# jiaowoguanren0615/Segmentation_Factory

Measured on AMD Instinct MI355X. Metric: images/sec/GPU fwd+bwd SegFormer-B0 512x512 bf16; mIoU parity vs CPU ref, higher is better.
Workload: dtype bf16; 1 GPU; SegFormer-B0 (MiT-B0 + 768-wide SegFormerHead as the reference builds it), 150 classes, 512x512, full train step (zero_grad+fwd+CE/Dice+bwd+AGC/AdamW); per_gpu_batch=256, global_batch=256, parallelism=dp1, fp8=False, inputs=resident in HBM in the captured step's input buffers (zero-copy feed), launch=hipGraph(zero_grad+fwd+loss+bwd+grad gather) + RCCL all-reduce + fused AGC/AdamW

## Files before the change

### include/segfac.h

```cpp
#ifndef SEGFAC_H
#define SEGFAC_H
#include <stdint.h>

#ifdef __cplusplus
extern "C" {
#endif

#define SEGF_F32 0
#define SEGF_BF16 1
#define SEGF_ERR_SHAPE (-1)
#define SEGF_ERR_DTYPE (-2)
#define SEGF_ERR_WORKSPACE (-3)

const char* segf_version(void);

int segf_cast(const void* src, int src_dt, void* dst, int dst_dt, int64_t n, void* stream);
int segf_cast2d(const void* src, int src_dt, int64_t ld_src, void* dst, int dst_dt, int64_t ld_dst, int64_t rows, int64_t cols,
                void* stream);
int segf_permute021(const void* in, int in_dt, void* out, int out_dt, int64_t A, int64_t Bd, int64_t Cd,
                    int64_t ld_out, void* stream);
typedef struct SegfPrepItem {
    const void* src; void* dst;
    int64_t rows, cols, ld_src, ld_dst, pb, pc;
    int32_t op, src_dt, dst_dt, reserved;
// ... 105 lines not shown
int segf_bn_cls_bwd_supported(int dt, int64_t M, int C, int K, int64_t rows_per_sample);
int64_t segf_bn_cls_bwd_ws(int64_t M, int C, int64_t rows_per_sample);
int segf_bn_cls_bwd(int dt, int64_t M, int C, int K, const void* dy, int64_t ldy, const void* w, int64_t ldw, const void* x,
                    const float* mean, const float* rstd, const float* gamma, const float* beta, int act,
                    const float* chan_scale, int64_t rows_per_sample, int eval_mode, void* dx, float* dgamma, float* dbeta,
                    float* ws, void* stream);
int segf_bn_cls_bwd_dw_supported(int dt, int64_t M, int C, int K, int64_t rows_per_sample, int C1);
int64_t segf_bn_cls_bwd_dw_ws(int64_t M, int C, int64_t rows_per_sample);
int segf_bn_cls_bwd_dw(int dt, int64_t M, int C, int K, const void* dy, int64_t ldy, const void* w, int64_t ldw, const void* x,
                       const float* mean, const float* rstd, const float* gamma, const float* beta, int act,
                       const float* chan_scale, int64_t rows_per_sample, int eval_mode, void* dx, float* dgamma,
                       float* dbeta, float* ws, const void* x1, int64_t ldx1, int C1, float* dG, void* stream);
int64_t segf_bn_cls_bwd_full_ws(int64_t M, int C, int K, int64_t rows_per_sample);
int segf_bn_cls_bwd_full(int dt, int64_t M, int C, int K, const void* dy, int64_t ldy, const void* w, int64_t ldw, const void* x,
                         const float* mean, const float* rstd, const float* gamma, const float* beta, int act,
                         const float* chan_scale, int64_t rows_per_sample, int eval_mode, void* dx, float* dgamma, float* dbeta,
                         float* ws, const void* x1, int64_t ldx1, int C1, float* dG, float* dwcls, void* stream);

int64_t segf_grn_ws(int B, int64_t rows_per_sample, int C, int bwd);
int segf_grn_fwd(int dt, int B, int64_t rows_per_sample, int C, const void* x, const float* gamma, const float* beta, void* y,
                 float* a_scratch, float* sumsq_out, float* ws, int pre_gelu, void* stream);
int segf_grn_bwd(int dt, int B, int64_t rows_per_sample, int C, const void* x, const void* dy, const float* gamma,
                 const float* sumsq_saved, void* dx, float* dgamma, float* dbeta, float* ws, int pre_gelu, void* stream);

int segf_attention_fwd(int dt, int B, int heads, int N, int Nkv, int hd, const void* q, int64_t ldq,
                       const void* k, int64_t ldk, const void* v, int64_t ldv, float scale,
                       void* o, int64_t ldo, float* lse, void* stream);
int64_t segf_attention_bwd_ws(int B, int heads, int N, int Nkv, int hd);
int segf_attention_bwd(int dt, int B, int heads, int N, int Nkv, int hd, const void* q, int64_t ldq,
                       const void* k, int64_t ldk, const void* v, int64_t ldv, float scale,
                       const void* o, int64_t ldo, const void* d_o, int64_t lddo, const float* lse,
                       void* dq, int64_t lddq, void* dk, int64_t lddk, void* dv, int64_t lddv,
                       float* ws, void* stream);

int segf_group_attention_supported(int dt, int B, int H, int W, int heads, int hd, int G, int interval, int lda);
int segf_group_attention_fwd(int dt, int B, int H, int W, int heads, int hd, int G, int interval, int lda, const void* qkv,
                             int64_t ldqkv, const float* bias, float scale, void* o, int64_t ldo, float* lse, void* stream);
int64_t segf_group_attention_bwd_ws(int B, int H, int W, int heads, int hd, int G, int interval, int lda);
int segf_group_attention_bwd(int dt, int B, int H, int W, int heads, int hd, int G, int interval, int lda, const void* qkv,
                             int64_t ldqkv, const float* bias, float scale, const void* d_o, int64_t lddo, const float* lse,
                             void* dqkv, int64_t lddqkv, float* dbias, float* ws, void* stream);

int segf_dwconv3x3_gelu_fwd(int dt, int B, int H, int W, int C, const void* x, const float* w ,
                            const float* bias, int apply_gelu, void* y, void* stream);
int64_t segf_dwconv3x3_bwd_ws(int B, int H, int W, int C);
int segf_dwconv3x3_bwd_blocks(int dt, int B, int H, int W, int C);
int segf_dwconv3x3_gelu_bwd(int dt, int B, int H, int W, int C, const void* x, const float* w, const float* bias,
                            int apply_gelu, const void* dy, void* du, void* dx, float* dw, float* db,
                            float* ws, void* stream);
int segf_dwconv3x3_gelu_bwd_fc2_supported(int dt, int B, int H, int W, int C_hidden, int C_in);
int segf_dwconv3x3_gelu_bwd_fc2(int dt, int B, int H, int W, int C_hidden, int C_in, const void* f, const float* w9,
                                const float* bias, const void* dys, int64_t ld_dys, const void* w2, void* du, void* dx,
                                float* dw, float* db, float* ws, void* stream);

int segf_dwconv7x7_fwd(int dt, int B, int H, int W, int C, const void* x, const float* wt, const float* bias, void* y,
                       void* stream);
int64_t segf_dwconv7x7_bwd_ws(int B, int H, int W, int C);
int segf_dwconv7x7_bwd(int dt, int B, int H, int W, int C, const void* x, const float* wt, const void* dy, void* dx,
                       float* dw, float* db, float* ws, void* stream);

int segf_conv3x3_fwd_splitk(int mode, int B, int H, int W, int Cin, int Cout);
int segf_conv3x3_pick_splitk(int Cin, int Cout, int64_t P);
int segf_conv3x3(int mode, int B, int H, int W, int Cin, int Cout, const void* x, int64_t ldx, const void* w, int64_t ldw,
                 void* y, int y_dt, int64_t ldy, const float* bias, int split_k, float* ws, void* stream);

int segf_conv3x3_dil_live_taps(int H, int W, int dilation, int* taps );
int segf_conv3x3_dil_supported(int dt, int mode, int B, int H, int W, int Cin, int Cout, int dilation);
int segf_conv3x3_dil_pick_splitk(int B, int H, int W, int Cin, int Cout, int dilation);
int segf_conv3x3_dil(int dt, int mode, int B, int H, int W, int Cin, int Cout, int dilation, const void* x, int64_t ldx,
                     const void* w, int64_t ldw, void* y, int64_t ldy, int split_k, float* ws, void* stream);

int segf_gelu(int dt, int mode, const void* u, const void* dy, void* y, int64_t n, void* stream);
int segf_rowdot(const float* a, int64_t lda, const float* b, int64_t ldb, const float* extra_a, const float* extra_b,
                float* out, int64_t rows, int64_t cols, void* stream);
int segf_adaptive_avgpool(int dt, int bwd, int B, int H, int W, int C, int S, const void* in, void* out, void* stream);

int segf_im2col(int dt, int in_nchw_f32, int B, int H, int W, int Cin, int kh, int kw, int stride, int pad,
                int Ho, int Wo, const void* x, void* col, int64_t ldcol, void* stream);
int segf_col2im(int dt, int B, int H, int W, int Cin, int kh, int kw, int stride, int pad,
                int Ho, int Wo, const void* dcol, int64_t ldcol, void* dx, void* stream);

int segf_bilinear_fwd(int dt, int B, int h, int w, int C, const void* in, int64_t ldi,
                      int H, int W, void* out, int64_t ldo, int align_corners, void* stream);
int segf_bilinear_bwd(int dt, int B, int h, int w, int C, void* din, int64_t ldi,
                      int H, int W, const void* dout, int64_t ldo, int align_corners, void* stream);
int segf_bilinear_bwd_248(int dt, int B, int H, int W, int C, const void* dout, int64_t ldo, void* d2, void* d4, void* d8,
                          void* stream);
int segf_upsample_add(int dt, int B, int H, int W, int C, const void* base, int64_t ldb, int nsrc,
                      const void* src0, int h0, int w0, int64_t ld0, const void* src1, int h1, int w1, int64_t ld1,
                      const void* src2, int h2, int w2, int64_t ld2, void* out, int64_t ldo, int align_corners, void* stream);
int64_t segf_upsample_add_stats_ws(int B, int H, int W, int C);
int segf_upsample_add_stats(int dt, int B, int H, int W, int C, const void* base, int64_t ldb, int nsrc,
                            const void* src0, int h0, int w0, int64_t ld0, const void* src1, int h1, int w1, int64_t ld1,
                            const void* src2, int h2, int w2, int64_t ld2, void* out, int64_t ldo, int align_corners,
                            float* sums, float* ws, void* stream);
int segf_fuse_map_248_supported(int dt, int B, int H, int W, int C, int C1);
int64_t segf_fuse_map_248_ws(int B, int H, int W, int C);
int segf_fuse_map_248(int B, int H, int W, int C, int C1, const void* x1, int64_t ldx1, const void* g1, int64_t ldg,
                      const void* t2, int64_t ld2, const void* t3, int64_t ld3, const void* t4, int64_t ld4,
                      void* out, int64_t ldo, float* sums, float* ws, void* stream);
int segf_bn_stats_from_sums(const float* sums, int64_t rows, int C, float* mean, float* rstd, float* running_mean,
                            float* running_var, float momentum, float eps, void* stream);
int segf_nearest_up(int dt, int bwd, int B, int h, int w, int C, int H, int W, const void* in, const void* base, void* out,
                    void* stream);
int segf_bilinear_to_nchw_f32(int dt, int B, int h, int w, int C, const void* in, int64_t ldi,
                              int H, int W, float* out, void* stream);
// ... 70 lines not shown
```

### segmentation_factory_amd/csrc/conv.hip

```cpp
#include <stdlib.h>
#include "colreduce.h"

#define DW_PIX 4

template <typename T, int MODE>
__global__ void __launch_bounds__(256) dwconv3x3_kernel(const T* __restrict__ x, const float* __restrict__ w,
                                                         const float* __restrict__ bias, int apply_gelu,
                                                         const T* __restrict__ dy, T* __restrict__ y, int B, int H, int W, int C) {
    const int nchunk = C / 8;
    const int wg = (W + DW_PIX - 1) / DW_PIX;
    const int units = B * H * wg;
    const int64_t g = (int64_t)xcd_block() * 256 + threadIdx.x;
    const int ustep = (int)(((int64_t)gridDim.x * 256) / nchunk);
    const int c0 = (int)(g % nchunk) * 8;
    f32x2_t wk[9][4], bs[4];
#pragma unroll
    for (int jj = 0; jj < 4; ++jj) {
#pragma unroll
        for (int kk = 0; kk < 9; ++kk) {
            const int ks = MODE == 1 ? 8 - kk : kk;
            wk[kk][jj] = f32x2_t{w[(c0 + 2 * jj) * 9 + ks], w[(c0 + 2 * jj + 1) * 9 + ks]};
        }
        bs[jj] = (MODE != 1 && bias) ? f32x2_t{bias[c0 + 2 * jj], bias[c0 + 2 * jj + 1]} : f32x2_t{0.f, 0.f};
    }
// ... 311 lines not shown
                load_row(yin + 2, rawb[(j + 2) % 3]);
                load_grow(yin + 1, dysb[(j + 2) % 3]);
                const bool vy = yin >= 0 && yin < H && yin <= yb;
#pragma unroll
                for (int cx = 0; cx < DW_PIX + 2; ++cx) {
                    f32x2_t v[2];
                    unpack4v(curc[cx], vy && cok[cx], v);
#pragma unroll
                    for (int kx = 0; kx < 3; ++kx) {
                        const int p = cx - kx;
                        if (p >= 0 && p < DW_PIX) {
#pragma unroll
                            for (int jj = 0; jj < 2; ++jj) {
                                P[p][jj] = wk[6 + kx][jj] * v[jj] + P[p][jj];
                                Cc[p][jj] = wk[3 + kx][jj] * v[jj] + Cc[p][jj];
                                N[p][jj] = wk[kx][jj] * v[jj] + N[p][jj];
                            }
                        }
                    }
                }
                const int yo = yin - 1;
                if (yo >= ya && yo < yb) {
                    dwf_f32x4 dgf[4];
#pragma unroll
                    for (int jm = 0; jm < 4; ++jm) {
                        dgf[jm] = dwf_f32x4{0.f, 0.f, 0.f, 0.f};
#pragma unroll
                        for (int s = 0; s < KS; ++s)
                            dgf[jm] = __builtin_amdgcn_mfma_f32_16x16x32_bf16(__builtin_bit_cast(dwf_bf16x8, gcurc[s]), Bf[jm][s], dgf[jm], 0, 0, 0);
                    }
                    T* orow = yo_b + (int64_t)yo * W * C;
#pragma unroll
                    for (int h = 0; h < DW_PIX / 2; ++h) {
                        f32x2_t a8[4] = {P[2 * h][0], P[2 * h][1], P[2 * h + 1][0], P[2 * h + 1][1]};
                        Raw4<T> q0, q1;
                        q0.u.x = pack2bf(dgf[0][2 * h], dgf[1][2 * h]); q0.u.y = pack2bf(dgf[2][2 * h], dgf[3][2 * h]);
                        q1.u.x = pack2bf(dgf[0][2 * h + 1], dgf[1][2 * h + 1]); q1.u.y = pack2bf(dgf[2][2 * h + 1], dgf[3][2 * h + 1]);
                        f32x2_t gy[4], g0[2], g1[2];
                        unpack4v(q0, true, g0); unpack4v(q1, true, g1);
                        gy[0] = g0[0]; gy[1] = g0[1]; gy[2] = g1[0]; gy[3] = g1[1];
                        gelu_erf8<true>(a8, gy);
                        const f32x2_t o0[2] = {a8[0], a8[1]}, o1[2] = {a8[2], a8[3]};
                        if (cok[2 * h + 1]) store4v(orow + coff[2 * h + 1], o0);
                        if (cok[2 * h + 2]) store4v(orow + coff[2 * h + 2], o1);
                    }
                }
#pragma unroll
                for (int p = 0; p < DW_PIX; ++p) { P[p][0] = bs[0]; P[p][1] = bs[1]; }
            }
        }
    }
}

static inline int dw_blocks(int B, int H, int W, int C) {
    return colfixed_blocks((int64_t)B * H * ((W + DW_PIX - 1) / DW_PIX), C / 8, 8, 16384);
}

extern "C" int segf_dwconv3x3_gelu_fwd(int dt, int B, int H, int W, int C, const void* x, const float* w, const float* bias,
                                       int apply_gelu, void* y, void* stream) {
    if (B <= 0 || H <= 0 || W <= 0) return 0;
    if (C <= 0 || C % 8 != 0 || ((uintptr_t)x % 16) || ((uintptr_t)y % 16)) return SEGF_ERR_SHAPE;
    if ((int64_t)B * H * W >= (1ll << 31)) return SEGF_ERR_SHAPE;
    hipStream_t st = (hipStream_t)stream;
    const int blocks = dw_blocks(B, H, W, C);
    SEGF_DISPATCH_DT(dt, T, {
        if (dw_use_walk()) dw_walk_launch<T, 0>(st, (const T*)x, w, bias, apply_gelu, (const T*)nullptr, (T*)y, B, H, W, C);
        else
        hipLaunchKernelGGL((dwconv3x3_kernel<T, 0>), dim3(blocks), dim3(256), 0, st, (const T*)x, w, bias, apply_gelu,
                           (const T*)nullptr, (T*)y, B, H, W, C);
    })
    SEGF_CHECK_LAUNCH();
    return 0;
}

#define DWG_MAX_BLOCKS 1024
struct DwgPlan { int ch, rl, slabs, nblk, units_per_blk; };
static inline DwgPlan dwg_plan(int B, int H, int W, int C) {
    DwgPlan p;
    const int nchunk = C / 8;
    p.ch = nchunk < 256 ? nchunk : 256;
    p.rl = 256 / p.ch;
    p.slabs = (nchunk + p.ch - 1) / p.ch;
    const int64_t units = (int64_t)B * H * ((W + DW_PIX - 1) / DW_PIX);
    int64_t want = cdiv64(units, (int64_t)p.rl * 4);
    int cap = DWG_MAX_BLOCKS / p.slabs;
    if (cap < 1) cap = 1;
    p.nblk = (int)(want < 1 ? 1 : (want > cap ? cap : want));
    p.units_per_blk = (int)cdiv64(units, p.nblk);
    return p;
}

template <typename T>
__global__ void __launch_bounds__(256) dwconv3x3_wgrad_kernel(const T* __restrict__ x, const T* __restrict__ du,
                                                               float* __restrict__ partial, int B, int H, int W, int C, int ch,
                                                               int rl, int units_per_blk) {
    __shared__ float red[256 * 8];
    const int tx = threadIdx.x % ch, ty = threadIdx.x / ch;
    const int chunk = blockIdx.y * ch + tx;
    const int c0 = chunk * 8;
    const bool active = ty < rl && c0 < C;
    const int wg = (W + DW_PIX - 1) / DW_PIX;
    const int units = B * H * wg;
    float acc[10][8];
#pragma unroll
    for (int o = 0; o < 10; ++o)
#pragma unroll
        for (int j = 0; j < 8; ++j) acc[o][j] = 0.f;
    (void)units_per_blk;
    if (active) {
        for (int u = (int)xcd_block() * rl + ty; u < units; u += (int)gridDim.x * rl) {
            const int xg = u % wg;
            const int t = u / wg;
            const int yy = t % H;
            const int b = t / H;
            const int x0 = xg * DW_PIX;
            Raw8<T> graw[DW_PIX], vraw[3][DW_PIX + 2];
#pragma unroll
            for (int p = 0; p < DW_PIX; ++p) {
                const int xp = x0 + p < W ? x0 + p : W - 1;
                graw[p] = load8_raw<T>(du + (((int64_t)b * H + yy) * W + xp) * C + c0);
            }
#pragma unroll
            for (int ky = 0; ky < 3; ++ky) {
// ... 955 lines not shown
```

### segmentation_factory_amd/csrc/policy.h

```cpp
#pragma once

#define SEGF_POLICY_TABLE(X)                                                                                                             \
                                                                                                   \
    X(gemm_no_big, "SEGFAC_GEMM_NO_BIG", 0, "never take the 256 x 256-tile kernel (gemm_bf16_big_kernel): everything on the 128-tile one") \
    X(gemm_no_skinny, "SEGFAC_GEMM_NO_SKINNY", 0, "no streaming products for K, N <= 128 (gemm_skinny_kernel and its relatives)")        \
    X(gemm_no_skinny_rows, "SEGFAC_GEMM_NO_SKINNY_ROWS", 0, "the [tokens x 32] -> 768 projection on gemm_skinny_kernel instead of the whole-row form") \
    X(gemm_no_skinny_k, "SEGFAC_GEMM_NO_SKINNY_K", 0, "no K-split streaming product for 32- / 64-wide outputs (gemm_skinny_k_kernel)")  \
    X(gemm_no_dw_skinny, "SEGFAC_GEMM_NO_DW_SKINNY", 0, "small-output weight gradients on the tiled split-K kernel instead of gemm_dw_skinny_kernel") \
    X(gemm_no_narrow, "SEGFAC_GEMM_NO_NARROW", 0, "256-tile kernel: full 128 x 64 wave tiles also for outputs <= 160 wide (bit-identical results)") \
    X(gemm_no_deep, "SEGFAC_GEMM_NO_DEEP", 0, "256-tile forward: one K step of operand loads in flight instead of two")                  \
    X(gemm_no_deep128, "SEGFAC_GEMM_NO_DEEP128", 0, "128-tile kernel: one K step in flight instead of two")                              \
    X(gemm_no_fastload, "SEGFAC_GEMM_NO_FASTLOAD", 0, "guarded tile loads everywhere (no workgroup-uniform guard-free full-K-step loads)") \
    X(gemm_no_tr, "SEGFAC_GEMM_NO_TR", 0, "debugging: reduction-major fragments by scalar LDS reads instead of ds_read_b64_tr_b16; disables every kernel built on the transposed read") \
    X(gemm_no_pro, "SEGFAC_GEMM_NO_PRO", 0, "segf_gemm_pro_supported answers 0: BatchNorm + ReLU + Dropout2d are applied by their own pass") \
    X(gemm_no_fused_db, "SEGFAC_GEMM_NO_FUSED_DB", 0, "bias gradient as its own column-sum launch instead of riding on the weight-gradient product") \
    X(no_grouped_dw, "SEGFAC_NO_GROUPED_DW", 0, "segf_gemm_dw_db_grouped runs its members one by one")                                   \
    X(dw_no_xcd_slabs, "SEGFAC_DW_NO_XCD_SLABS", 0, "split-K weight gradients (128-tile kernel) in hardware workgroup order instead of one K slab per XCD")                \
    X(dw_no_shared_split, "SEGFAC_DW_NO_SHARED_SPLIT", 0, "grouped weight gradients keep their per-layer slice counts (also read by the host layer)") \
    X(no_wide_reduce, "SEGFAC_NO_WIDE_REDUCE", 0, "split-K partials of large outputs summed by the 16 x 16 form instead of whole rows")   \
    X(no_reduce4, "SEGFAC_NO_REDUCE4", 0, "split-K reduce: one output per thread instead of four (bitwise the same sums)")               \
    X(gemm_f32_no_mfma, "SEGFAC_GEMM_F32_NO_MFMA", 0, "fp32 storage (exact-parity mode, evaluate): products on the vector FMA kernel instead of the f32 matrix instruction") \
    X(gemm8_linear, "SEGFAC_GEMM8_LINEAR", 1, "0: plain nn.Linear products never take the eight-phase kernel (the 256 / 128 tile kernels as in r04)") \
    X(gemm8_linear_min_tiles, "SEGFAC_GEMM8_LINEAR_MIN_TILES", 128, "fewest 256 x 256 tiles for which a K >= 2048 nn.Linear product takes the eight-phase kernel (192 for shorter K)") \
    X(gemm8_linear_min_fill, "SEGFAC_GEMM8_LINEAR_MIN_FILL", 60, "smallest share (percent) of the launched 256 x 256 tiles that must be output for an nn.Linear product with ragged last tiles to take the eight-phase kernel") \
    X(gemm8_linear_min_k, "SEGFAC_GEMM8_LINEAR_MIN_K", 256, "shortest reduction for which an nn.Linear product takes the eight-phase kernel (its 12-load prologue and drain against K / 64 tiles)") \
    X(gemm8_dw, "SEGFAC_GEMM8_DW", 1, "0: nn.Linear weight gradients never take the eight-phase kernel below 65536 tokens (the grouped 128-tile kernel as in r04)") \
    X(gemm8_dw_min_gflop, "SEGFAC_GEMM8_DW_MIN_GFLOP", 100, "smallest nn.Linear weight gradient (GFLOP; both feature counts multiples of 256, >= 256 FLOP per operand byte) that takes the eight-phase kernel + a column-sum pass instead of the grouped 128-tile kernel") \
    X(gemm8_linear_min_gflop, "SEGFAC_GEMM8_LINEAR_MIN_GFLOP", 36, "smallest nn.Linear product (GFLOP, K >= 512; 100 for shorter K) that takes the eight-phase kernel") \
                                 \
    X(no_gemm8, "SEGFAC_NO_GEMM8", 0, "no eight-phase kernel at all (gemm8_kernel): the two-phase 256-tile kernel everywhere")           \
    X(no_gemm8t, "SEGFAC_NO_GEMM8T", 0, "no eight-phase kernel for weight gradients (reduction-major operands)")                         \
    X(conv_no_fwd_split, "SEGFAC_CONV_NO_FWD_SPLIT", 0, "3 x 3 forward / data gradient with few output tiles: no split over the (channel block, tap) walk") \
    X(g8_stagger, "SEGFAC_G8_STAGGER", -1, "eight-phase kernel: 1 = wave groups one barrier apart, 0 = lockstep, -1 = staggered for bf16 and the per-device choice (segf_gemm8_option) for fp8") \
    X(no_fp8, "SEGFAC_NO_FP8", 0, "segf_gemm_fp8_supported answers 0 (block-scaled 128-tile fp8 GEMM)")                                  \
    X(no_fp8_conv, "SEGFAC_NO_FP8_CONV", 0, "segf_conv3x3_fp8*_supported answer 0")                                                      \
    X(no_fp8_wgrad, "SEGFAC_NO_FP8_WGRAD", 0, "fp8 3 x 3 convolutions keep a bf16 weight gradient")                                      \
    X(no_fp8_linear, "SEGFAC_NO_FP8_LINEAR", 0, "segf_linear_fp8_supported answers 0")                                                   \
                                                                             \
    X(dilconv_no_cull, "SEGFAC_DILCONV_NO_CULL", 0, "dilated 3 x 3 convolution: all nine taps are walked, with zero loads where a tap leaves the image, instead of the live taps only") \
                                                                            \
    X(attn_no_mfma, "SEGFAC_ATTN_NO_MFMA", 0, "attention on the VALU reference kernels (attention.hip) also in bf16")                    \
    X(attn_f32_no_mfma, "SEGFAC_ATTN_F32_NO_MFMA", 0, "fp32 attention forward on the vector kernel (one query per lane) instead of the f32 matrix instruction") \
    X(attn64_prescale, "SEGFAC_ATTN64_PRESCALE", 0, "head dim 64, >= 128 keys: scale log2(e) rides on the Q fragments (bf16(q c), one more rounding per q element) and -max / -lse are the score accumulators' initial values, instead of one multiply-add per score: forward + query-side backward, +8 % / +2 % per kernel, attention error x 1.2 - 2.3") \
    X(attn64_dkv_rows, "SEGFAC_ATTN64_DKV_ROWS", 128, "head dim 64, >= 128 keys, key-side backward: query rows per staged Q / dO tile and barrier (128, 64 or 32: the same arithmetic, bit for bit)") \
    X(attn_no_fused_bwd, "SEGFAC_ATTN_NO_FUSED_BWD", 0, "head dim 32, <= 256 keys: query-side + key-side backward kernels instead of the one-kernel backward") \
                                                                                \
    X(dw_no_walk, "SEGFAC_DW_NO_WALK", 0, "depthwise 3 x 3: the round-1 strip kernels instead of the vertical-walk kernels")             \
    X(dw_walk_rows, "SEGFAC_DW_WALK_ROWS", 0, "depthwise 3 x 3 walk: rows per segment (0 = chosen from the map size)")                   \
    X(dw_no_small, "SEGFAC_DW_NO_SMALL", 0, "depthwise 3 x 3 backward of small maps: three passes instead of the one-launch LDS form")   \
    X(dw_small_always, "SEGFAC_DW_SMALL_ALWAYS", 0, "... the one-launch form beyond one round of workgroups as well")                    \
    X(ffn_bwd_fused, "SEGFAC_FFN_BWD_FUSED", 1, "Mix-FFN backward, fc2's data gradient formed inside pass A of the depthwise backward (segf_dwconv3x3_gelu_bwd_fc2_supported): 0 = never, 1 = from 131072 token rows on, 2 = wherever the shape has the kernel") \
                                                           \
    X(no_fuse_map, "SEGFAC_NO_FUSE_MAP", 0, "folded SegFormerHead map: streaming product + VALU upsample-add instead of fuse_map_kernel") \
    X(no_bwd248_mfma, "SEGFAC_NO_BWD248_MFMA", 0, "transposed 1/2-1/4-1/8 resizes on the VALU kernel instead of fuse_map_bwd_kernel")    \
    X(upadd_generic, "SEGFAC_UPADD_GENERIC", 0, "upsample-add: the generic per-source kernels also for the 2-4-8 pyramid")               \
    X(no_head_fused, "SEGFAC_NO_HEAD_FUSED", 0, "segf_bn_cls_bwd_supported answers 0: classifier data gradient and BatchNorm backward as separate passes") \
    X(no_head_fused_dw, "SEGFAC_NO_HEAD_FUSED_DW", 0, "the folded head's stage-1 weight gradient does not ride on pass 2 of the fused BatchNorm backward") \
                                                                                 \
    X(loss_no_band, "SEGFAC_LOSS_NO_BAND", 0, "CE / Dice forward and backward on the tile kernels instead of the band sweep")            \
    X(loss_no_band_fwd, "SEGFAC_LOSS_NO_BAND_FWD", 0, "... the forward only")                                                             \
    X(loss_band_rows, "SEGFAC_LOSS_BAND_ROWS", 0, "band sweep: rows per segment (0 = 16)")                                               \
    X(loss_no_mfma, "SEGFAC_LOSS_NO_MFMA", 0, "ratio-4 loss kernels on the VALU cells form (fp32 storage)")                              \
    X(loss_no_retry, "SEGFAC_LOSS_NO_RETRY", 0, "no exact per-pixel retry pass behind the flagged cells")                                \
    X(loss_no_lse, "SEGFAC_LOSS_NO_LSE", 0, "the backward recomputes the softmax normalisation instead of taking the forward's per-pixel log-sum") \
                                                                                                 \
    X(no_wide_finalize, "SEGFAC_NO_WIDE_FINALIZE", 0, "column-reduction finalize: one output per thread instead of four (bitwise the same sums)") \
                                                                                 \
    X(no_ln_patch, "SEGFAC_NO_LN_PATCH", 0, "[host] MiT blocks: im2col / col2im around the spatial-reduction conv instead of the patch-major LayerNorm output") \
    X(no_scaled_ln_bwd, "SEGFAC_NO_SCALED_LN_BWD", 0, "[host] DropPath backward as its own scale_rows launch instead of riding on the LayerNorm backward") \
    X(no_deferred_dw, "SEGFAC_NO_DEFERRED_DW", 0, "[host] weight gradients issued layer by layer inside the captured step (no grouped launches)") \
    X(no_deferred_finalize, "SEGFAC_NO_DEFERRED_FINALIZE", 0, "[host] LayerNorm dgamma / dbeta finalizes issued one by one")              \
    X(no_head_fused_cw, "SEGFAC_NO_HEAD_FUSED_CW", 0, "[host] the classifier's weight gradient as its own product instead of riding on pass 1 of the fused BatchNorm backward") \
    X(no_bwd248, "SEGFAC_NO_BWD248", 0, "[host] folded head backward: three segf_bilinear_bwd launches instead of the one-pass segf_bilinear_bwd_248") \
    X(no_gelu_grn, "SEGFAC_NO_GELU_GRN", 0, "[host] ConvNeXtV2 blocks: GELU as its own pass in front of the GRN kernels")                \
    X(no_weight_shadow, "SEGFAC_NO_WEIGHT_SHADOW", 0, "[host] captured step: weights cast to bf16 per use instead of one cast of the flat buffer") \
    X(no_derived_weights, "SEGFAC_NO_DERIVED_WEIGHTS", 0, "[host] captured step: derived weight layouts built in front of each layer instead of one grouped launch")

struct SegfPolicy {
#define SEGF_POLICY_FIELD(field, env, def, doc) int field;
    SEGF_POLICY_TABLE(SEGF_POLICY_FIELD)
#undef SEGF_POLICY_FIELD
    int g8_stagger_fp8;
};

const SegfPolicy& segf_policy();
#define POL(field) (segf_policy().field)

struct SegfTrace {
    int on;
    int dry;
    int n;
    const char* names[256];
    const char* where[256];
};
SegfTrace& segf_trace();
void segf_trace_note(const char* kernel_text, const char* where);
```

### segmentation_factory_amd/functional.py

```python
import contextlib

import torch
from torch.autograd import Function

from . import hip


def _rowmajor(t):
    return t if t.stride(-1) == 1 else t.contiguous()


_SHADOW = None


class shadow_scope:
    def __init__(self, table):
        self.table = table

    def __enter__(self):
        global _SHADOW
        self.prev, _SHADOW = _SHADOW, self.table
        return self

    def __exit__(self, *exc):
# ... 770 lines not shown
        return dqkv, dbias, None, None, None, None, None, None, None


def group_attention(qkv, bias, B, H, W, heads, G, interval, lda):
    return GroupAttentionFn.apply(qkv, bias, B, H, W, heads, G, interval, bool(lda))


@direct_grads(1, 2)
class DWConvGeluFn(Function):

    @staticmethod
    def forward(ctx, x, weight, bias, B, H, W, apply_gelu):
        x = x if x.is_contiguous() else x.contiguous()
        Cc = x.shape[1]
        w9 = weight.detach().reshape(Cc, 9).contiguous()
        b = bias.detach().contiguous() if bias is not None else None
        y = hip.dwconv3x3_gelu_fwd(x, w9, b, B, H, W, Cc, apply_gelu)
        ctx.save_for_backward(x, w9, b)
        ctx.meta = (B, H, W, Cc, apply_gelu, weight.shape)
        return y

    @staticmethod
    def backward(ctx, dy):
        x, w9, b = ctx.saved_tensors
        B, H, W, Cc, apply_gelu, wshape = ctx.meta
        dy = dy if dy.is_contiguous() else dy.contiguous()
        gw, gb = gslot(ctx, 1), (gslot(ctx, 2) if b is not None else None)
        q = _FIN_QUEUE
        if q is not None and gw is not None and gb is not None and gb.data_ptr() == gw.data_ptr() + 4 * gw.numel() and gw.is_contiguous():
            slots = ctx._gslots
            dx, item = hip.dwconv3x3_gelu_bwd(x, w9, b, dy, B, H, W, Cc, apply_gelu, dw_out=gw, db_out=gb, defer=True)
            q.append((item, (slots[1], slots[2])))
            if len(q) >= FIN_QUEUE_MAX:
                _flush_finalizes()
            return dx, None, None, None, None, None, None
        dx, dw, db = hip.dwconv3x3_gelu_bwd(x, w9, b, dy, B, H, W, Cc, apply_gelu, dw_out=gw, db_out=gb)
        return dx, dw.view(wshape), (db if b is not None else None), None, None, None, None


def dwconv3x3_gelu(x, weight, bias, B, H, W, apply_gelu=True):
    return DWConvGeluFn.apply(x, weight, bias, B, H, W, apply_gelu)


@direct_grads(1, 2, 3, 4)
class DWConvGeluLinearFn(Function):

    @staticmethod
    def forward(ctx, x, weight2, bias2, weight, bias, B, H, W, residual, rscale):
        x = x if x.is_contiguous() else x.contiguous()
        M, Cc = x.shape
        N = weight2.shape[0]
        w9 = weight.detach().reshape(Cc, 9).contiguous()
        b = bias.detach().contiguous()
        g = hip.dwconv3x3_gelu_fwd(x, w9, b, B, H, W, Cc, True)
        w2 = _w(weight2.reshape(N, -1), x.dtype)
        y = hip.gemm(0, g, w2, M, N, Cc, bias=bias2.detach(), residual=residual, rscale=rscale, rows_per_group=H * W)
        ctx.save_for_backward(x, w9, b, g, w2, rscale)
        ctx.meta = (B, H, W, Cc, N, M, weight.shape, weight2.shape, residual is not None)
        return y

    @staticmethod
    def backward(ctx, dy):
        x, w9, b, g, w2, rscale = ctx.saved_tensors
        B, H, W, Cc, N, M, wshape, w2shape, has_res = ctx.meta
        dy = _rowmajor(dy)
        dys = dy
        if rscale is not None:
            dys = _take_scaled(dy, rscale, H * W)
            if dys is None:
                dys = hip.scale_rows(dy, rscale, H * W)
        dw2 = db2 = None
        if not _queue_dw(ctx, dys, g, N, Cc, M):
            dw2, db2 = hip.gemm_dw_db(dys, g, N, Cc, M, split_k=_splitk(N, Cc, M), out=gslot(ctx, 1, (N, Cc)), db_out=gslot(ctx, 2))
            dw2 = dw2.view(w2shape)
        gw, gb = gslot(ctx, 3), gslot(ctx, 4)
        dres = dy if (has_res and ctx.needs_input_grad[8]) else None
        q = _FIN_QUEUE
        if q is not None and gw is not None and gb is not None and gb.data_ptr() == gw.data_ptr() + 4 * gw.numel() and gw.is_contiguous():
            slots = ctx._gslots
            dx, item = hip.dwconv3x3_gelu_bwd_fc2(x, w9, b, dys, w2, B, H, W, Cc, N, dw_out=gw, db_out=gb, defer=True)
            q.append((item, (slots[3], slots[4])))
            if len(q) >= FIN_QUEUE_MAX:
                _flush_finalizes()
            return dx, dw2, db2, None, None, None, None, None, dres, None
        dx, dw, db = hip.dwconv3x3_gelu_bwd_fc2(x, w9, b, dys, w2, B, H, W, Cc, N, dw_out=gw, db_out=gb)
        return dx, dw2, db2, dw.view(wshape), db, None, None, None, dres, None


def dwconv3x3_gelu_linear_ok(x, weight2, bias2, weight, bias, B, H, W):
    if not (x.is_cuda and x.dtype == torch.bfloat16 and torch.is_grad_enabled() and x.requires_grad):
        return False
    if bias is None or bias2 is None or not all(p.requires_grad for p in (weight2, bias2, weight, bias)):
        return False
    return hip.dwconv3x3_gelu_bwd_fc2_supported(x.dtype, B, H, W, x.shape[1], weight2.shape[0])


def dwconv3x3_gelu_linear(x, weight2, bias2, weight, bias, B, H, W, residual=None, rscale=None):
    y = DWConvGeluLinearFn.apply(x, weight2, bias2, weight, bias, B, H, W, residual, rscale)
    if rscale is not None:
        y._segf_dp = (rscale, H * W)
    return y


@direct_grads(1, 2)
class BatchNormActFn(Function):

    @staticmethod
    def forward(ctx, x, gamma, beta, running_mean, running_var, training, momentum, eps, act, chan_scale, rows_per_sample,
                pre_sums=None):
        x = x if x.is_contiguous() else x.contiguous()
        g, b = gamma.detach().contiguous(), beta.detach().contiguous()
        if training and pre_sums is not None:
            mean, rstd = hip.bn_stats_from_sums(pre_sums, x.shape[0], running_mean, running_var, momentum, eps)
        elif training:
            mean, rstd = hip.bn_stats(x, running_mean, running_var, momentum, eps)
        else:
            mean = running_mean.detach().clone()
            rstd = torch.rsqrt(running_var.detach() + eps)
        y = hip.bn_apply(x, mean, rstd, g, b, act, chan_scale, rows_per_sample or 1)
        ctx.save_for_backward(x, mean, rstd, g, b, chan_scale)
        ctx.meta = (act, rows_per_sample or 1, not training)
        return y

    @staticmethod
    def backward(ctx, dy):
        x, mean, rstd, g, b, chan_scale = ctx.saved_tensors
        act, rps, eval_mode = ctx.meta
        dy = dy if dy.is_contiguous() else dy.contiguous()
        dx, dg, db = hip.bn_bwd(x, dy, mean, rstd, g, b, act, chan_scale, rps, eval_mode)
        return dx, dg, db, None, None, None, None, None, None, None, None, None


def batch_norm_act(x, gamma, beta, running_mean, running_var, training, momentum=0.1, eps=1e-5, act=1, chan_scale=None,
                   rows_per_sample=None, pre_sums=None):
    return BatchNormActFn.apply(x, gamma, beta, running_mean, running_var, training, momentum, eps, act, chan_scale,
                                rows_per_sample, pre_sums)


@direct_grads(1, 2, 11, 12)
# ... 702 lines not shown
```

### segmentation_factory_amd/hip.py

```python
import ctypes as C
import os
import re

import torch

_HERE = os.path.dirname(os.path.abspath(__file__))
LIB_PATH = os.environ.get('SEGFAC_HIP_LIB') or os.path.join(_HERE, 'libsegfac_hip.so')
HEADER_PATH = os.path.normpath(os.path.join(_HERE, '..', 'include', 'segfac.h'))
F32, BF16 = 0, 1
ERR_SHAPE = -1
_lib = None

_i, _l, _f, _p = C.c_int, C.c_int64, C.c_float, C.c_void_p
_SCALAR = {'int': _i, 'int32_t': _i, 'int64_t': _l, 'float': _f}
_POINTEE = {'void', 'char', 'int', 'int32_t', 'int64_t', 'uint8_t', 'uint64_t', 'float'}


def _ctype(ctype, where, structs):
    t = re.sub(r'\bconst\b', ' ', ctype).replace('*', ' * ').split()
    if t and all(w == '*' for w in t[1:]):
        base, stars = t[0], len(t) - 1
        if stars == 0 and base in _SCALAR:
            return _SCALAR[base]
        if stars == 1 and base == 'char':
# ... 794 lines not shown
    dq = torch.empty((B * N, heads * hd), dtype=q.dtype, device=q.device)
    ws = _f32(lib().segf_attention_bwd_ws(B, heads, N, Nkv, hd), q.device)
    _chk(lib().segf_attention_bwd(dt_of(q), B, heads, N, Nkv, hd, _ptr(q), q.stride(0), _ptr(k), k.stride(0), _ptr(v),
                                  v.stride(0), scale, _ptr(o), o.stride(0), _ptr(d_o), d_o.stride(0), _ptr(lse),
                                  _ptr(dq), dq.stride(0), _ptr(dk), dk.stride(0), _ptr(dv), dv.stride(0), _ptr(ws),
                                  _stream()), 'segf_attention_bwd')
    return dq


def _group_attention_check(t, B, H, W, heads, G, interval, lda):
    if G * G <= 64 and not lib().segf_group_attention_supported(dt_of(t), B, H, W, heads, 32, G, interval, int(lda)):
        raise RuntimeError(f'group attention: no kernel for a {H} x {W} map, batch {B}, {heads} heads of 32, groups of {G} x {G} '
                           f'({"LDA" if lda else "SDA"}, interval {interval}): sizes must be positive and B * H * W below 2^29')
    if G * G > 64:
        raise RuntimeError(f'group attention: no kernel for groups of {G} x {G} = {G * G} tokens ({"LDA" if lda else "SDA"}, interval '
                           f'{interval}) on a {H} x {W} map, batch {B}, {heads} heads of 32: a group holds at most 64 tokens '
                           f'(there is no fallback path)')


def group_attention_fwd(qkv, bias, B, H, W, heads, G, interval, lda, scale):
    _need_cuda(qkv, bias)
    _group_attention_check(qkv, B, H, W, heads, G, interval, lda)
    rows = B * H * W
    assert qkv.shape[0] == rows and qkv.stride(1) == 1 and bias.is_contiguous() and bias.dtype == torch.float32
    assert qkv.shape[1] >= 3 * heads * 32, f'qkv has {qkv.shape[1]} columns, {heads} heads of 32 need {3 * heads * 32}'
    assert tuple(bias.shape) == (heads, G * G, G * G), (tuple(bias.shape), heads, G)
    o = torch.empty((rows, heads * 32), dtype=qkv.dtype, device=qkv.device)
    lse = torch.empty((heads, rows), dtype=torch.float32, device=qkv.device)
    _chk(lib().segf_group_attention_fwd(dt_of(qkv), B, H, W, heads, 32, G, interval, int(lda), _ptr(qkv), qkv.stride(0), _ptr(bias),
                                        scale, _ptr(o), o.stride(0), _ptr(lse), _stream()), 'segf_group_attention_fwd')
    return o, lse


def group_attention_bwd(qkv, bias, d_o, lse, B, H, W, heads, G, interval, lda, scale):
    _need_cuda(qkv, bias, d_o)
    _group_attention_check(qkv, B, H, W, heads, G, interval, lda)
    assert qkv.shape[1] >= 3 * heads * 32 and d_o.shape[1] >= heads * 32 and d_o.stride(1) == 1
    dqkv = torch.empty((B * H * W, 3 * heads * 32), dtype=qkv.dtype, device=qkv.device)
    dbias = torch.empty((heads, G * G, G * G), dtype=torch.float32, device=qkv.device)
    ws = _f32(lib().segf_group_attention_bwd_ws(B, H, W, heads, 32, G, interval, int(lda)), qkv.device)
    _chk(lib().segf_group_attention_bwd(dt_of(qkv), B, H, W, heads, 32, G, interval, int(lda), _ptr(qkv), qkv.stride(0), _ptr(bias),
                                        scale, _ptr(d_o), d_o.stride(0), _ptr(lse), _ptr(dqkv), dqkv.stride(0), _ptr(dbias), _ptr(ws),
                                        _stream()), 'segf_group_attention_bwd')
    return dqkv, dbias


def dwconv3x3_gelu_fwd(x, w9, bias, B, H, W, Cc, apply_gelu=True):
    y = torch.empty_like(x)
    _chk(lib().segf_dwconv3x3_gelu_fwd(dt_of(x), B, H, W, Cc, _ptr(x), _ptr(w9), _ptr(bias), int(apply_gelu), _ptr(y),
                                       _stream()), 'segf_dwconv3x3_gelu_fwd')
    return y


def dwconv3x3_gelu_bwd(x, w9, bias, dy, B, H, W, Cc, apply_gelu=True, dw_out=None, db_out=None, defer=False):
    du = torch.empty_like(x)
    dx = torch.empty_like(x)
    if defer:
        assert dw_out.dtype == db_out.dtype == torch.float32 and dw_out.is_contiguous() and dw_out.numel() == 9 * Cc
        assert db_out.numel() == Cc and db_out.data_ptr() == dw_out.data_ptr() + 36 * Cc
        ws = _f32(lib().segf_dwconv3x3_bwd_ws(B, H, W, Cc), x.device)
        _chk(lib().segf_dwconv3x3_gelu_bwd(dt_of(x), B, H, W, Cc, _ptr(x), _ptr(w9), _ptr(bias), int(apply_gelu), _ptr(dy),
                                           _ptr(du), _ptr(dx), None, None, _ptr(ws), _stream()), 'segf_dwconv3x3_gelu_bwd')
        return dx, (ws, int(lib().segf_dwconv3x3_bwd_blocks(dt_of(x), B, H, W, Cc)), 10 * Cc, dw_out, Cc)
    dw = dw_out if dw_out is not None else torch.empty((Cc, 9), dtype=torch.float32, device=x.device)
    db = db_out if db_out is not None else torch.empty(Cc, dtype=torch.float32, device=x.device)
    assert dw.is_contiguous() and dw.numel() == Cc * 9 and db.is_contiguous() and db.numel() == Cc and dw.dtype == db.dtype == torch.float32
    ws = _f32(lib().segf_dwconv3x3_bwd_ws(B, H, W, Cc), x.device)
    _chk(lib().segf_dwconv3x3_gelu_bwd(dt_of(x), B, H, W, Cc, _ptr(x), _ptr(w9), _ptr(bias), int(apply_gelu), _ptr(dy),
                                       _ptr(du), _ptr(dx), _ptr(dw), _ptr(db), _ptr(ws), _stream()),
         'segf_dwconv3x3_gelu_bwd')
    return dx, dw, db


def dwconv3x3_gelu_bwd_fc2_supported(dtype, B, H, W, Cc, Cin):
    dt = BF16 if dtype == torch.bfloat16 else F32
    return bool(lib().segf_dwconv3x3_gelu_bwd_fc2_supported(dt, B, H, W, Cc, Cin))


def dwconv3x3_gelu_bwd_fc2(x, w9, bias, dys, w2, B, H, W, Cc, Cin, dw_out=None, db_out=None, defer=False, return_du=False):
    _need_cuda(x, dys, w2)
    assert x.dtype == dys.dtype == w2.dtype == torch.bfloat16 and x.is_contiguous() and w2.is_contiguous()
    assert dys.shape == (B * H * W, Cin) and dys.stride(1) == 1 and w2.shape == (Cin, Cc)
    du = torch.empty_like(x)
    dx = torch.empty_like(x)
    ws = _f32(lib().segf_dwconv3x3_bwd_ws(B, H, W, Cc), x.device)
    if defer:
        assert dw_out.dtype == db_out.dtype == torch.float32 and dw_out.is_contiguous() and dw_out.numel() == 9 * Cc
        assert db_out.numel() == Cc and db_out.data_ptr() == dw_out.data_ptr() + 36 * Cc
        blocks = int(lib().segf_dwconv3x3_bwd_blocks(dt_of(x), B, H, W, Cc))
        _chk(lib().segf_dwconv3x3_gelu_bwd_fc2(BF16, B, H, W, Cc, Cin, _ptr(x), _ptr(w9), _ptr(bias), _ptr(dys), dys.stride(0), _ptr(w2),
                                               _ptr(du), _ptr(dx), None, None, _ptr(ws), _stream()), 'segf_dwconv3x3_gelu_bwd_fc2')
        out = (dx, (ws, blocks, 10 * Cc, dw_out, Cc))
        return out + (du,) if return_du else out
    dw = dw_out if dw_out is not None else torch.empty((Cc, 9), dtype=torch.float32, device=x.device)
    db = db_out if db_out is not None else torch.empty(Cc, dtype=torch.float32, device=x.device)
    assert dw.is_contiguous() and dw.numel() == Cc * 9 and db.is_contiguous() and db.numel() == Cc and dw.dtype == db.dtype == torch.float32
    _chk(lib().segf_dwconv3x3_gelu_bwd_fc2(BF16, B, H, W, Cc, Cin, _ptr(x), _ptr(w9), _ptr(bias), _ptr(dys), dys.stride(0), _ptr(w2),
                                           _ptr(du), _ptr(dx), _ptr(dw), _ptr(db), _ptr(ws), _stream()), 'segf_dwconv3x3_gelu_bwd_fc2')
    return (dx, dw, db, du) if return_du else (dx, dw, db)


def dwconv7x7_fwd(x, wt49, bias, B, H, W, Cc):
    y = torch.empty_like(x)
    _chk(lib().segf_dwconv7x7_fwd(dt_of(x), B, H, W, Cc, _ptr(x), _ptr(wt49), _ptr(bias), _ptr(y), _stream()),
         'segf_dwconv7x7_fwd')
    return y
# ... 317 lines not shown
```

Measured before the change: 4757 images/sec.

## Fuse Mix-FFN fc2 GEMM into depthwise 3x3 GELU forward walk kernel

Adds a forward kernel that computes the depthwise 3x3 conv plus GELU and, on the same pass, runs the fc2 projection with MFMA from an LDS slab of the just-computed activations. It also adds bias, the optional residual and the per-sample scale before writing the output. This removes the separate GEMM launch and its re-read of the hidden activation g from HBM; g is still written for backward. The price is heavier kernels with LDS-staged weights and extra registers, which may lower occupancy. It is gated by a policy knob and a minimum row count, and only covers bf16 shapes with C_in of 32 or 64.

```diff
diff --git a/include/segfac.h b/include/segfac.h
--- a/include/segfac.h
+++ b/include/segfac.h
@@ -181,6 +181,10 @@
 int segf_dwconv3x3_gelu_bwd_fc2(int dt, int B, int H, int W, int C_hidden, int C_in, const void* f, const float* w9,
                                 const float* bias, const void* dys, int64_t ld_dys, const void* w2, void* du, void* dx,
                                 float* dw, float* db, float* ws, void* stream);
+int segf_dwconv3x3_gelu_fwd_fc2_supported(int dt, int B, int H, int W, int C_hidden, int C_in);
+int segf_dwconv3x3_gelu_fwd_fc2(int dt, int B, int H, int W, int C_hidden, int C_in, const void* f, const float* w9,
+                                const float* bias, const void* w2, const float* b2, const void* residual, const float* rscale,
+                                void* g, void* y, void* stream);
 
 int segf_dwconv7x7_fwd(int dt, int B, int H, int W, int C, const void* x, const float* wt, const float* bias, void* y,
                        void* stream);
diff --git a/segmentation_factory_amd/csrc/conv.hip b/segmentation_factory_amd/csrc/conv.hip
--- a/segmentation_factory_amd/csrc/conv.hip
+++ b/segmentation_factory_amd/csrc/conv.hip
@@ -387,6 +387,198 @@
     }
 }
 
+template <int KS, int CL>
+__global__ void __launch_bounds__(256, 2) dwconv3x3_walk_lin_kernel(const bf16_t* __restrict__ x, const float* __restrict__ w,
+                                                                     const float* __restrict__ bias, bf16_t* __restrict__ y,
+                                                                     const bf16_t* __restrict__ w2, const float* __restrict__ b2,
+                                                                     const bf16_t* __restrict__ res, const float* __restrict__ rscale,
+                                                                     bf16_t* __restrict__ out, int B, int H, int W, int R, int nseg) {
+    static_assert((KS == 4 || KS == 8) && KS % CL == 0, "C_hidden = 128 or 256, whole chains");
+    typedef bf16_t T;
+    constexpr int C = 32 * KS, NCHUNK = C / 4, SPW = 64 / NCHUNK;
+    constexpr int N = C / 4, NT = N / 16;
+    constexpr int TPS = 4 * SPW, RPG = 16 / TPS;
+    constexpr int SROW = 2 * C + 16;
+    __shared__ __attribute__((aligned(16))) unsigned char slab_all[4][16 * SROW];
+    __shared__ int tokrow_all[4][16], toksmp_all[4][16];
+    __shared__ __attribute__((aligned(16))) unsigned char wlds[NT * KS * 1024];
+    const int lane = threadIdx.x & 63, wave = threadIdx.x >> 6;
+    const int mi = lane & 15, gq = lane >> 4;
+    const int half = lane / NCHUNK, chunk = lane % NCHUNK;
+    const int c0 = chunk * 4;
+    unsigned char* slab = slab_all[wave];
+    int* tokrow = tokrow_all[wave];
+    int* toksmp = toksmp_all[wave];
+    const int wg = (W + DW_PIX - 1) / DW_PIX;
+    const int units = B * nseg * wg;
+    const int wv = __builtin_amdgcn_readfirstlane((int)(xcd_block() * 4 + wave));
+    const int ustep = (int)gridDim.x * 4 * SPW;
+    f32x2_t wk[9][2], bs[2];
+#pragma unroll
+    for (int jj = 0; jj < 2; ++jj) {
+#pragma unroll
+        for (int kk = 0; kk < 9; ++kk) wk[kk][jj] = f32x2_t{w[(c0 + 2 * jj) * 9 + kk], w[(c0 + 2 * jj + 1) * 9 + kk]};
+        bs[jj] = f32x2_t{bias[c0 + 2 * jj], bias[c0 + 2 * jj + 1]};
+    }
+    for (int f = wave; f < NT * KS; f += 4) {
+        const int nt = f / KS, s = f % KS;
+        const int n = 32 * (nt >> 1) + 8 * (mi >> 2) + 4 * (nt & 1) + (mi & 3);
+        *reinterpret_cast<uint4*>(wlds + f * 1024 + lane * 16) = *reinterpret_cast<const uint4*>(w2 + (int64_t)n * C + 32 * s + 8 * gq);
+    }
+    __syncthreads();
+    const int steps = (R + 2 + 2) / 3;
+    for (int ub = wv * SPW; ub < units; ub += ustep) {
+        const bool live = ub + half < units;
+        const int u = live ? ub + half : units - 1;
+        const int xg = u % wg;
+        const int t = u / wg;
+        const int seg = t % nseg;
+        const int b = t / nseg;
+        const int x0 = xg * DW_PIX;
+        const int ya = seg * R, yb = ya + R < H ? ya + R : H;
+        const T* xb = x + (int64_t)b * H * W * C + c0;
+        T* yo_b = y + (int64_t)b * H * W * C + c0;
+        int coff[DW_PIX + 2];
+        bool cok[DW_PIX + 2];
+#pragma unroll
+        for (int cx = 0; cx < DW_PIX + 2; ++cx) {
+            const int ix = x0 + cx - 1;
+            cok[cx] = ix >= 0 && ix < W;
+            coff[cx] = (ix < 0 ? 0 : (ix >= W ? W - 1 : ix)) * C;
+        }
+        f32x2_t acc[3][DW_PIX][2];
+#pragma unroll
+        for (int a = 0; a < 3; ++a)
+#pragma unroll
+            for (int p = 0; p < DW_PIX; ++p) { acc[a][p][0] = bs[0]; acc[a][p][1] = bs[1]; }
+        Raw4<T> rawb[3][DW_PIX + 2];
+        auto load_row = [&](int yin, Raw4<T> (&dst)[DW_PIX + 2]) {
+            const int yc = yin < 0 ? 0 : (yin >= H ? H - 1 : yin);
+            const T* row = xb + (int64_t)yc * W * C;
+#pragma unroll
+            for (int cx = 0; cx < DW_PIX + 2; ++cx) dst[cx] = load4_raw<T>(row + coff[cx]);
+        };
+        load_row(ya - 1, rawb[0]);
+        load_row(ya, rawb[1]);
+        int yin = ya - 1;
+        int rel = -2;
+        for (int st = 0; st < steps; ++st) {
+#pragma unroll
+            for (int j = 0; j < 3; ++j, ++yin, ++rel) {
+                f32x2_t (&P)[DW_PIX][2] = acc[j % 3];
+                f32x2_t (&Cc)[DW_PIX][2] = acc[(j + 1) % 3];
+                f32x2_t (&N_)[DW_PIX][2] = acc[(j + 2) % 3];
+                Raw4<T> (&curc)[DW_PIX + 2] = rawb[j % 3];
+                load_row(yin + 2, rawb[(j + 2) % 3]);
+                const bool vy = yin >= 0 && yin < H && yin <= yb;
+#pragma unroll
+                for (int cx = 0; cx < DW_PIX + 2; ++cx) {
+                    f32x2_t v[2];
+                    unpack4v(curc[cx], vy && cok[cx], v);
+#pragma unroll
+                    for (int kx = 0; kx < 3; ++kx) {
+                        const int p = cx - kx;
+                        if (p >= 0 && p < DW_PIX) {
+#pragma unroll
+                            for (int jj = 0; jj < 2; ++jj) {
+                                P[p][jj] = wk[6 + kx][jj] * v[jj] + P[p][jj];
+                                Cc[p][jj] = wk[3 + kx][jj] * v[jj] + Cc[p][jj];
+                                N_[p][jj] = wk[kx][jj] * v[jj] + N_[p][jj];
+                            }
+                        }
+                    }
+                }
+                if (rel >= 0 && rel < R) {
+                    const int yo = yin - 1;
+                    const bool rok = live && yo < yb;
+                    const int rstep = rel % RPG;
+                    T* orow = yo_b + (int64_t)yo * W * C;
+                    unsigned char* srow = slab + (rstep * TPS + half * DW_PIX) * SROW + c0 * 2;
+#pragma unroll
+                    for (int h = 0; h < DW_PIX / 2; ++h) {
+                        f32x2_t a8[4] = {P[2 * h][0], P[2 * h][1], P[2 * h + 1][0], P[2 * h + 1][1]};
+                        gelu_erf8<false>(a8, nullptr);
+                        uint2 q0, q1;
+                        q0.x = pack2bf(a8[0].x, a8[0].y); q0.y = pack2bf(a8[1].x, a8[1].y);
+                        q1.x = pack2bf(a8[2].x, a8[2].y); q1.y = pack2bf(a8[3].x, a8[3].y);
+                        if (rok && cok[2 * h + 1]) *reinterpret_cast<uint2*>(orow + coff[2 * h + 1]) = q0;
+                        if (rok && cok[2 * h + 2]) *reinterpret_cast<uint2*>(orow + coff[2 * h + 2]) = q1;
+                        *reinterpret_cast<uint2*>(srow + (2 * h) * SROW) = q0;
+                        *reinterpret_cast<uint2*>(srow + (2 * h + 1) * SROW) = q1;
+                    }
+                    if (chunk < DW_PIX) {
+                        const int slot = rstep * TPS + half * DW_PIX + chunk;
+                        const bool tv = rok && x0 + chunk < W;
+                        tokrow[slot] = tv ? (b * H + yo) * W + x0 + chunk : -1;
+                        toksmp[slot] = b;
+                    }
+                    if (rstep == RPG - 1 || rel == R - 1) {
+                        __builtin_amdgcn_fence(__ATOMIC_ACQ_REL, "wavefront");
+                        __builtin_amdgcn_wave_barrier();
+                        const int trow = tokrow[mi];
+                        const bool tv = mi / TPS <= rstep && trow >= 0;
+                        const int64_t m = tv ? trow : 0;
+                        dwf_u32x4 rres[NT / 2];
+                        float rs = 1.f;
+                        if (res) {
+#pragma unroll
+                            for (int q = 0; q < NT / 2; ++q) rres[q] = *reinterpret_cast<const dwf_u32x4*>(res + m * N + 32 * q + 8 * gq);
+                            if (rscale) rs = rscale[tv ? toksmp[mi] : 0];
+                        }
+                        float bv[NT][4];
+#pragma unroll
+                        for (int nt = 0; nt < NT; ++nt) {
+#pragma unroll
+                            for (int r = 0; r < 4; ++r) bv[nt][r] = b2[32 * (nt >> 1) + 8 * gq + 4 * (nt & 1) + r];
+                        }
+                        dwf_f32x4 pacc[NT];
+#pragma unroll
+                        for (int c = 0; c < KS / CL; ++c) {
+                            dwf_u32x4 xa[CL];
+#pragma unroll
+                            for (int s = 0; s < CL; ++s) xa[s] = *reinterpret_cast<const dwf_u32x4*>(slab + mi * SROW + (32 * (CL * c + s) + 8 * gq) * 2);
+#pragma unroll
+                            for (int nt = 0; nt < NT; ++nt) {
+                                dwf_f32x4 part = dwf_f32x4{0.f, 0.f, 0.f, 0.f};
+#pragma unroll
+                                for (int s = 0; s < CL; ++s) {
+                                    const dwf_bf16x8 wf = __builtin_bit_cast(dwf_bf16x8, *reinterpret_cast<const uint4*>(wlds + (nt * KS + CL * c + s) * 1024 + lane * 16));
+                                    part = __builtin_amdgcn_mfma_f32_16x16x32_bf16(wf, __builtin_bit_cast(dwf_bf16x8, xa[s]), part, 0, 0, 0);
+                                }
+                                if (c == 0) pacc[nt] = part;
+                                else
+#pragma unroll
+                                    for (int r = 0; r < 4; ++r) pacc[nt][r] = pacc[nt][r] + part[r];
+                            }
+                        }
+#pragma unroll
+                        for (int q = 0; q < NT / 2; ++q) {
+                            float v[8];
+#pragma unroll
+                            for (int r = 0; r < 4; ++r) { v[r] = pacc[2 * q][r] + bv[2 * q][r]; v[4 + r] = pacc[2 * q + 1][r] + bv[2 * q + 1][r]; }
+                            if (res) {
+                                const dwf_u32x4 wr = rres[q];
+#pragma unroll
+                                for (int jr = 0; jr < 4; ++jr) {
+                                    v[2 * jr] = __uint_as_float(wr[jr] << 16) + rs * v[2 * jr];
+                                    v[2 * jr + 1] = __uint_as_float(wr[jr] & 0xffff0000u) + rs * v[2 * jr + 1];
+                                }
+                            }
+                            uint4 o;
+                            o.x = pack2bf(v[0], v[1]); o.y = pack2bf(v[2], v[3]); o.z = pack2bf(v[4], v[5]); o.w = pack2bf(v[6], v[7]);
+                            if (tv) *reinterpret_cast<uint4*>(out + m * N + 32 * q + 8 * gq) = o;
+                        }
+                        __builtin_amdgcn_fence(__ATOMIC_ACQ_REL, "wavefront");
+                        __builtin_amdgcn_wave_barrier();
+                    }
+                }
+#pragma unroll
+                for (int p = 0; p < DW_PIX; ++p) { P[p][0] = bs[0]; P[p][1] = bs[1]; }
+            }
+        }
+    }
+}
+
 static inline int dw_blocks(int B, int H, int W, int C) {
     return colfixed_blocks((int64_t)B * H * ((W + DW_PIX - 1) / DW_PIX), C / 8, 8, 16384);
 }
@@ -404,6 +596,45 @@
         hipLaunchKernelGGL((dwconv3x3_kernel<T, 0>), dim3(blocks), dim3(256), 0, st, (const T*)x, w, bias, apply_gelu,
                            (const T*)nullptr, (T*)y, B, H, W, C);
     })
+    SEGF_CHECK_LAUNCH();
+    return 0;
+}
+
+#define DW_LIN_MIN_ROWS 131072
+static inline bool dw_lin_shape_ok(int dt, int B, int H, int W, int C, int Cin) {
+    return dt == SEGF_BF16 && B > 0 && H > 0 && W > 0 && (Cin == 32 || Cin == 64) && C == 4 * Cin && (int64_t)B * H * W < (1ll << 31);
+}
+extern "C" int segf_dwconv3x3_gelu_fwd_fc2_supported(int dt, int B, int H, int W, int C_hidden, int C_in) {
+    if (!dw_lin_shape_ok(dt, B, H, W, C_hidden, C_in) || !dw_use_walk()) return 0;
+    const int pol = POL(ffn_fwd_lin);
+    if (pol <= 0) return 0;
+    if (pol >= 2) return 1;
+    return (int64_t)B * H * W >= DW_LIN_MIN_ROWS;
+}
+extern "C" int segf_dwconv3x3_gelu_fwd_fc2(int dt, int B, int H, int W, int C_hidden, int C_in, const void* f, const float* w9,
+                                           const float* bias, const void* w2, const float* b2, const void* residual,
+                                           const float* rscale, void* g, void* y, void* stream) {
+    if (B <= 0 || H <= 0 || W <= 0) return 0;
+    if (dt != SEGF_BF16) return SEGF_ERR_DTYPE;
+    if (!dw_lin_shape_ok(dt, B, H, W, C_hidden, C_in) || !dw_use_walk()) return SEGF_ERR_SHAPE;
+    if (((uintptr_t)f % 16) || ((uintptr_t)g % 16) || ((uintptr_t)w2 % 16) || ((uintptr_t)y % 16) || ((uintptr_t)residual % 16) || !bias || !b2)
+        return SEGF_ERR_SHAPE;
+    hipStream_t st = (hipStream_t)stream;
+    typedef bf16_t T;
+    const int C = C_hidden;
+    int R, nseg;
+    dw_walk_plan(H, R, nseg, (int64_t)B * ((W + DW_PIX - 1) / DW_PIX) * (C / 4));
+    const int64_t units = (int64_t)B * nseg * ((W + DW_PIX - 1) / DW_PIX);
+    const int blocks = colfixed_blocks(units, C / 4, 1, 32768);
+    if (C_in == 32)
+        hipLaunchKernelGGL((dwconv3x3_walk_lin_kernel<4, 4>), dim3(blocks), dim3(256), 0, st, (const T*)f, w9, bias, (T*)g, (const T*)w2, b2,
+                           (const T*)residual, rscale, (T*)y, B, H, W, R, nseg);
+    else if ((int64_t)B * H * W >= 65536 && !POL(gemm_no_skinny_k))
+        hipLaunchKernelGGL((dwconv3x3_walk_lin_kernel<8, 2>), dim3(blocks), dim3(256), 0, st, (const T*)f, w9, bias, (T*)g, (const T*)w2, b2,
+                           (const T*)residual, rscale, (T*)y, B, H, W, R, nseg);
+    else
+        hipLaunchKernelGGL((dwconv3x3_walk_lin_kernel<8, 8>), dim3(blocks), dim3(256), 0, st, (const T*)f, w9, bias, (T*)g, (const T*)w2, b2,
+                           (const T*)residual, rscale, (T*)y, B, H, W, R, nseg);
     SEGF_CHECK_LAUNCH();
     return 0;
 }
diff --git a/segmentation_factory_amd/csrc/policy.h b/segmentation_factory_amd/csrc/policy.h
--- a/segmentation_factory_amd/csrc/policy.h
+++ b/segmentation_factory_amd/csrc/policy.h
@@ -50,6 +50,7 @@
     X(dw_no_small, "SEGFAC_DW_NO_SMALL", 0, "depthwise 3 x 3 backward of small maps: three passes instead of the one-launch LDS form")   \
     X(dw_small_always, "SEGFAC_DW_SMALL_ALWAYS", 0, "... the one-launch form beyond one round of workgroups as well")                    \
     X(ffn_bwd_fused, "SEGFAC_FFN_BWD_FUSED", 1, "Mix-FFN backward, fc2's data gradient formed inside pass A of the depthwise backward (segf_dwconv3x3_gelu_bwd_fc2_supported): 0 = never, 1 = from 131072 token rows on, 2 = wherever the shape has the kernel") \
+    X(ffn_fwd_lin, "SEGFAC_FFN_FWD_LIN", 1, "Mix-FFN forward, fc2's output formed inside the depthwise walk (segf_dwconv3x3_gelu_fwd_fc2_supported): 0 = never, 1 = from 131072 token rows on, 2 = wherever the shape has the kernel") \
                                                            \
     X(no_fuse_map, "SEGFAC_NO_FUSE_MAP", 0, "folded SegFormerHead map: streaming product + VALU upsample-add instead of fuse_map_kernel") \
     X(no_bwd248_mfma, "SEGFAC_NO_BWD248_MFMA", 0, "transposed 1/2-1/4-1/8 resizes on the VALU kernel instead of fuse_map_bwd_kernel")    \
diff --git a/segmentation_factory_amd/functional.py b/segmentation_factory_amd/functional.py
--- a/segmentation_factory_amd/functional.py
+++ b/segmentation_factory_amd/functional.py
@@ -846,9 +846,12 @@
         N = weight2.shape[0]
         w9 = weight.detach().reshape(Cc, 9).contiguous()
         b = bias.detach().contiguous()
-        g = hip.dwconv3x3_gelu_fwd(x, w9, b, B, H, W, Cc, True)
         w2 = _w(weight2.reshape(N, -1), x.dtype)
-        y = hip.gemm(0, g, w2, M, N, Cc, bias=bias2.detach(), residual=residual, rscale=rscale, rows_per_group=H * W)
+        if _fwd_fc2_ok(x, w2, bias2, B, H, W, Cc, N, residual, rscale):
+            g, y = hip.dwconv3x3_gelu_fwd_fc2(x, w9, b, w2, bias2.detach(), B, H, W, Cc, N, residual=residual, rscale=rscale)
+        else:
+            g = hip.dwconv3x3_gelu_fwd(x, w9, b, B, H, W, Cc, True)
+            y = hip.gemm(0, g, w2, M, N, Cc, bias=bias2.detach(), residual=residual, rscale=rscale, rows_per_group=H * W)
         ctx.save_for_backward(x, w9, b, g, w2, rscale)
         ctx.meta = (B, H, W, Cc, N, M, weight.shape, weight2.shape, residual is not None)
         return y
@@ -879,6 +882,17 @@
             return dx, dw2, db2, None, None, None, None, None, dres, None
         dx, dw, db = hip.dwconv3x3_gelu_bwd_fc2(x, w9, b, dys, w2, B, H, W, Cc, N, dw_out=gw, db_out=gb)
         return dx, dw2, db2, dw.view(wshape), db, None, None, None, dres, None
+
+
+def _fwd_fc2_ok(x, w2, bias2, B, H, W, Cc, N, residual, rscale):
+    if not hip.dwconv3x3_gelu_fwd_fc2_supported(x.dtype, B, H, W, Cc, N):
+        return False
+    if not (w2.is_contiguous() and w2.data_ptr() % 16 == 0 and bias2.dtype == torch.float32 and bias2.is_contiguous()):
+        return False
+    if residual is not None and not (residual.dtype == x.dtype and residual.is_contiguous() and residual.shape == (B * H * W, N) and
+                                     residual.data_ptr() % 16 == 0):
+        return False
+    return rscale is None or (rscale.dtype == torch.float32 and rscale.is_contiguous() and rscale.numel() == B)
 
 
 def dwconv3x3_gelu_linear_ok(x, weight2, bias2, weight, bias, B, H, W):
diff --git a/segmentation_factory_amd/hip.py b/segmentation_factory_amd/hip.py
--- a/segmentation_factory_amd/hip.py
+++ b/segmentation_factory_amd/hip.py
@@ -870,6 +870,27 @@
     return y
 
 
+def dwconv3x3_gelu_fwd_fc2_supported(dtype, B, H, W, Cc, Cin):
+    dt = BF16 if dtype == torch.bfloat16 else F32
+    return bool(lib().segf_dwconv3x3_gelu_fwd_fc2_supported(dt, B, H, W, Cc, Cin))
+
+
+def dwconv3x3_gelu_fwd_fc2(x, w9, bias, w2, b2, B, H, W, Cc, Cin, residual=None, rscale=None):
+    _need_cuda(x, w2)
+    assert x.dtype == w2.dtype == torch.bfloat16 and x.is_contiguous() and w2.is_contiguous()
+    assert x.shape == (B * H * W, Cc) and w2.shape == (Cin, Cc) and bias.dtype == b2.dtype == torch.float32
+    assert bias.is_contiguous() and bias.numel() == Cc and b2.is_contiguous() and b2.numel() == Cin
+    if residual is not None:
+        assert residual.dtype == torch.bfloat16 and residual.shape == (B * H * W, Cin) and residual.is_contiguous()
+    if rscale is not None:
+        assert rscale.dtype == torch.float32 and rscale.is_contiguous() and rscale.numel() == B
+    g = torch.empty_like(x)
+    y = torch.empty((B * H * W, Cin), dtype=x.dtype, device=x.device)
+    _chk(lib().segf_dwconv3x3_gelu_fwd_fc2(BF16, B, H, W, Cc, Cin, _ptr(x), _ptr(w9), _ptr(bias), _ptr(w2), _ptr(b2), _ptr(residual),
+                                           _ptr(rscale), _ptr(g), _ptr(y), _stream()), 'segf_dwconv3x3_gelu_fwd_fc2')
+    return g, y
+
+
 def dwconv3x3_gelu_bwd(x, w9, bias, dy, B, H, W, Cc, apply_gelu=True, dw_out=None, db_out=None, defer=False):
     du = torch.empty_like(x)
     dx = torch.empty_like(x)
```

After: 4797 images/sec (median of 6 runs). Within noise of the previous version (+0.8%).
